# stone-d-chen/ffvvc

Measured on AMD Instinct MI355X. Metric: decoded frames/sec (4K/8K 10-bit VVC) per GPU, higher is better.
Workload: dtype u16

## Files before the change

ffvvc_amd/csrc/common.hpp:

```cpp
#pragma once
#include <hip/hip_runtime.h>
#include <stdint.h>
#include <stddef.h>
#include <stdio.h>
#include <stdlib.h>

#define VVC355_PB 128

namespace vvc355 { void hip_fail(const char *expr, int err, const char *what, const char *file, int line); }
#define HIP_CHECK(expr)                                                                         \
    do {                                                                                        \
        hipError_t e_ = (expr);                                                                 \
        if (e_ != hipSuccess)                                                                   \
            ::vvc355::hip_fail(#expr, (int)e_, hipGetErrorString(e_), __FILE__, __LINE__);      \
    } while (0)

namespace vvc355 {

template <int BD> struct Px       { using type = uint16_t; };
template <>       struct Px<8>    { using type = uint8_t;  };

__device__ __forceinline__ int clip3(int v, int lo, int hi) { return min(max(v, lo), hi); }
template <int BD> __device__ __forceinline__ int clip_px(int v) { return clip3(v, 0, (1 << BD) - 1); }
__device__ __forceinline__ int clip_intp2(int v, int p) { return clip3(v, -(1 << p), (1 << p) - 1); }
__device__ __forceinline__ int sign_of(int v) { return (v > 0) - (v < 0); }
__device__ __forceinline__ int ilog2(unsigned v) { return 31 - __clz(v | 1); }

#define VVC355_GLOBAL __attribute__((address_space(1)))
template <int N> struct RawBits;
template <> struct RawBits<1> { typedef uint8_t type; };
template <> struct RawBits<2> { typedef uint16_t type; };
template <> struct RawBits<4> { typedef uint32_t type; };
template <> struct RawBits<8> { typedef uint32_t type __attribute__((ext_vector_type(2))); };
template <> struct RawBits<16> { typedef uint32_t type __attribute__((ext_vector_type(4))); };
template <typename T> __device__ __forceinline__ T gld(const void *p)
{
    typedef typename RawBits<sizeof(T)>::type raw_t;
    const raw_t r = *(const VVC355_GLOBAL raw_t *)p;
    T v;
    __builtin_memcpy(&v, &r, sizeof(T));
    return v;
}
template <typename T> __device__ __forceinline__ void gst(void *p, T v)
{
    typedef typename RawBits<sizeof(T)>::type raw_t;
    raw_t r;
    __builtin_memcpy(&r, &v, sizeof(T));
    *(VVC355_GLOBAL raw_t *)p = r;
}

#define VVC355_CONST __attribute__((address_space(4)))
template <typename T> __device__ __forceinline__ T load_uniform(const T *p)
{
    static_assert(sizeof(T) % 4 == 0, "job descriptors are whole dwords");
    constexpr int N = sizeof(T) / 4;
    uint32_t w[N];
    const VVC355_CONST uint32_t *q = (const VVC355_CONST uint32_t *)p;
#pragma unroll
    for (int i = 0; i < N; i++) w[i] = q[i];
    T r;
    __builtin_memcpy(&r, w, sizeof(T));
    return r;
}

__device__ __forceinline__ ptrdiff_t row_off(int y, int stride) { return (ptrdiff_t)__mul24(y, stride); }

template <int BD> __device__ __forceinline__ int ld_px(const uint8_t *p, ptrdiff_t i)
{
    return ((const VVC355_GLOBAL typename Px<BD>::type *)p)[i];
}
template <int BD> __device__ __forceinline__ void st_px(uint8_t *p, ptrdiff_t i, int v)
{
    ((VVC355_GLOBAL typename Px<BD>::type *)p)[i] = (typename Px<BD>::type)v;
}

template <int BD> __device__ __forceinline__ int lmcs_fwd(const uint8_t *lut, int v)
{
    return lut ? (int)gld<typename Px<BD>::type>((const typename Px<BD>::type *)lut + v) : v;
}

template <typename T> __device__ __forceinline__ T gld_at(const uint8_t *base, uint32_t off) { return gld<T>(base + (size_t)off); }
template <typename T> __device__ __forceinline__ void gst_at(uint8_t *base, uint32_t off, T v) { gst<T>(base + (size_t)off, v); }

__device__ __forceinline__ int xcd_chunked(int b, int n)
{
    const int xcd = b & 7, idx = b >> 3, q = n >> 3, r = n & 7;
    return xcd * q + min(xcd, r) + idx;
}

__device__ __forceinline__ int xcd_grouped(int b, int n, int G)
{
    const int span = 8 * G, sg = b / span, r = b - sg * span;
    if ((sg + 1) * span > n)
        return b;
    return sg * span + (r & 7) * G + (r >> 3);
}

#define VVC355_BD_DISPATCH(bd, CALL)                         \
    do {                                                     \
        switch (bd) {                                        \
        case 8:  { constexpr int BD = 8;  CALL; } break;     \
        case 10: { constexpr int BD = 10; CALL; } break;     \
        case 12: { constexpr int BD = 12; CALL; } break;     \
        default:                                             \
            fprintf(stderr, "vvc_mi355: unsupported bit depth %d\n", (int)(bd)); abort(); \
        }                                                    \
    } while (0)

}
```

ffvvc_amd/csrc/inter_frame.hip:

```cpp
#include "common.hpp"
#include "inter_weight.hpp"
#include "runtime.hpp"
#include "../../include/vvc_mi355.h"

namespace vvc355 {

__global__ __launch_bounds__(256) void inter_build_kernel(const vvc355_inter_frame *__restrict__ fp)
{
    const vvc355_inter_frame f = load_uniform(fp);
    const int u = blockIdx.x * blockDim.x + threadIdx.x;
    if (u >= f.n_pus)
        return;
    const vvc355_inter_pu pu = ((const vvc355_inter_pu *)f.pus)[u];
    const vvc355_inter_slice *sl = (const vvc355_inter_slice *)f.slices + pu.slice;
    const vvc355_ref_pic *refs = (const vvc355_ref_pic *)f.refs;
    const MvFieldDev *mvf_tab = (const MvFieldDev *)f.mvf;
    vvc355_bipred_job *jl = (vvc355_bipred_job *)f.jobs_luma, *jc = (vvc355_bipred_job *)f.jobs_chroma;
    vvc355_bipred_result *rec = (vvc355_bipred_result *)f.records;
    const int sbw = pu.cb_width / pu.num_sb_x, sbh = pu.cb_height / pu.num_sb_y;
    const int tw = min(sbw, 16), th = min(sbh, 16);
    uint32_t job = pu.first_job;
    for (int sby = 0; sby < pu.num_sb_y; sby++)
        for (int sbx = 0; sbx < pu.num_sb_x; sbx++) {
            const int sx = pu.x0 + sbx * sbw, sy = pu.y0 + sby * sbh;
            const MvFieldDev mv = mvf_tab[(sy >> 2) * f.mvf_stride + (sx >> 2)];
            const bool bi = mv.pred_flag == 3;
            for (int ty = 0; ty < sbh; ty += th)
                for (int tx = 0; tx < sbw; tx += tw, job++) {
                    for (int c = 0; c < (f.chroma_format_idc ? 3 : 1); c++) {
                        const int hs = c ? f.hs : 0, vs = c ? f.vs : 0;
                        vvc355_bipred_job j = {};
                        const int x = (sx + tx) >> hs, y = (sy + ty) >> vs;
                        j.dst = f.dst[c] + (uint64_t)y * f.dst_stride[c] + ((uint64_t)x << f.pixel_shift);
                        j.dst_stride = f.dst_stride[c];
                        for (int l = 0; l < 2; l++) {
                            if (!(mv.pred_flag & (1 << l)))
                                continue;
                            const vvc355_ref_pic rp = refs[l * 16 + mv.ref_idx[l]];
                            (l ? j.ref1 : j.ref0) = rp.plane[c];
                            (l ? j.ref1_stride : j.ref0_stride) = rp.stride[c];
                            j.mv[2 * l] = mv.mv[l][0];
                            j.mv[2 * l + 1] = mv.mv[l][1];
                        }
                        j.rec = (uint64_t)(rec + job);
                        j.x = (int16_t)x; j.y = (int16_t)y; j.w = (int16_t)(tw >> hs); j.h = (int16_t)(th >> vs);
                        j.pic_w = (int16_t)(f.width >> hs); j.pic_h = (int16_t)(f.height >> vs);
                        j.chroma = c > 0; j.hs = f.hs; j.vs = f.vs;
                        j.dmvr = bi && pu.dmvr_flag;
                        j.bdof = !c && bi && pu.bdof_flag;
                        j.hf_idx = j.vf_idx = c ? 0 : pu.hpel_if_idx;
                        j.pred_flag = mv.pred_flag;
                        j.lmcs_lut = (!c && sl->lmcs_used && !pu.ciip_flag) ? f.lmcs_fwd_lut : 0;
                        set_pred_weight(j, derive_pred_weight(sl, mv, c, pu.dmvr_flag, pu.ciip_flag));
                        if (c == 0) jl[job] = j; else jc[2 * job + c - 1] = j;
                    }
                }
        }
}

__global__ __launch_bounds__(256) void inter_dmvr_info_kernel(const vvc355_inter_frame *__restrict__ fp)
{
    const vvc355_inter_frame f = load_uniform(fp);
    const int i = blockIdx.x * blockDim.x + threadIdx.x;
    if (i >= f.n_jobs)
        return;
    const vvc355_bipred_job *j = (const vvc355_bipred_job *)f.jobs_luma + i;
    if (!j->dmvr)
        return;
    const vvc355_bipred_result *r = (const vvc355_bipred_result *)f.records + i;
    const MvFieldDev *src = (const MvFieldDev *)f.mvf;
    MvFieldDev *dst = (MvFieldDev *)f.dmvr_mvf;
    MvFieldDev m = src[(j->y >> 2) * f.mvf_stride + (j->x >> 2)];
    m.mv[0][0] = r->mv[0]; m.mv[0][1] = r->mv[1]; m.mv[1][0] = r->mv[2]; m.mv[1][1] = r->mv[3];
    for (int y = j->y; y < j->y + j->h; y += 4)
        for (int x = j->x; x < j->x + j->w; x += 4)
            dst[(y >> 2) * f.mvf_stride + (x >> 2)] = m;
}

}

extern "C" {

void vvc355_inter_frame_build(void *stream, const vvc355_inter_frame *frame_dev, const vvc355_inter_frame *frame_host)
{
    if (frame_host->n_pus <= 0) return;
    hipLaunchKernelGGL(vvc355::inter_build_kernel, dim3((frame_host->n_pus + 255) / 256), dim3(256), 0, (hipStream_t)stream, frame_dev);
    HIP_CHECK(hipGetLastError());
}

void vvc355_inter_frame_pass(void *stream, int bd, const vvc355_inter_frame *frame_dev, const vvc355_inter_frame *frame_host)
{
    if (frame_host->n_pus <= 0 || frame_host->n_jobs <= 0) return;
    vvc355_inter_frame_build(stream, frame_dev, frame_host);
    vvc355_inter_frame_predict(stream, bd, frame_dev, frame_host);
}

void vvc355_inter_frame_predict(void *stream, int bd, const vvc355_inter_frame *frame_dev, const vvc355_inter_frame *frame_host)
{
    if (frame_host->n_pus <= 0 || frame_host->n_jobs <= 0) return;
    vvc355_bipred_batch(stream, bd, (const vvc355_bipred_job *)frame_host->jobs_luma, frame_host->n_jobs);
    if (frame_host->dmvr_mvf) {
        hipLaunchKernelGGL(vvc355::inter_dmvr_info_kernel, dim3((frame_host->n_jobs + 255) / 256), dim3(256), 0, (hipStream_t)stream, frame_dev);
        HIP_CHECK(hipGetLastError());
    }
    if (frame_host->chroma_format_idc)
        vvc355_bipred_chroma_batch(stream, bd, (const vvc355_bipred_job *)frame_host->jobs_chroma, 2 * frame_host->n_jobs);
}

}
```

ffvvc_amd/csrc/itx.hip:

```cpp
#include <type_traits>
#include "common.hpp"
#include "runtime.hpp"
#include "resid_math.hpp"
#include "../../include/vvc_mi355.h"
#include "stage_checks.hpp"

namespace vvc355 {

#define VVC355_TABLE(type, name, count) __device__ static const type d_tab_##name[count]
#include "tables.inc"
#undef VVC355_TABLE
#define VVC355_TABLE(type, name, count) static constexpr type c_##name[count]
#include "tables_small.inc"
#undef VVC355_TABLE
__host__ __device__ constexpr int level_scale_of(int rect, int rem)
{
    return rect ? (rem == 0 ? 57 : rem == 1 ? 64 : rem == 2 ? 72 : rem == 3 ? 80 : rem == 4 ? 90 : 102)
                : (rem == 0 ? 40 : rem == 1 ? 45 : rem == 2 ? 51 : rem == 3 ? 57 : rem == 4 ? 64 : 72);
}
static constexpr unsigned long long kDiag4X = 0x3323213210210100ull, kDiag4Y = 0x3231230123012010ull;
constexpr bool itx_small_tables_match()
{
    for (int r = 0; r < 2; r++)
        for (int q = 0; q < 6; q++)
// ... 408 lines not shown
            } else {
#pragma unroll
                for (int q = 0; q < PER; q++) {
                    const int o = e0 + q;
                    if (o < n)
                        st_px<BD>(dst + (ptrdiff_t)(o >> job.log2_w) * job.dst_stride, o & (w - 1), clip_px<BD>((int)pred[q] + r[q]));
                }
            }
        }
    }
}

template <int BD, int NT, int CAP, typename... Lv>
__global__ __launch_bounds__(256) void itx_kernel(const vvc355_itx_job *__restrict__ jobs, int n_jobs, Lv... lv)
{
    constexpr bool PACKED = sizeof...(Lv) > 0;
    constexpr int TBS = 256 / NT;
    __shared__ __attribute__((aligned(16))) int buf_all[TBS][CAP];
    __shared__ __attribute__((aligned(16))) int tmp_all[TBS][CAP];
    __shared__ int8_t cos_lds[256];
    cos_lds[threadIdx.x] = d_tab_dct2_cos[threadIdx.x];
    __syncthreads();
    const int sub = threadIdx.x / NT, tid = threadIdx.x % NT;
    const int ji = blockIdx.x * TBS + sub;
    if (ji >= n_jobs)
        return;
    vvc355_itx_job job = jobs[ji];
    resolve_type(job);
    if (job.log2_w + job.log2_h > __builtin_ctz(CAP))
        return;
    if constexpr (PACKED) {
        const LvSrc ls = lv_src(lv...);
        const vvc355_tb_levels r = ls.lv[ji];
        itx_generic_block<BD, NT, CAP, true>(job, buf_all[sub], tmp_all[sub], cos_lds, tid, &r, ls.levels);
    } else {
        itx_generic_block<BD, NT, CAP>(job, buf_all[sub], tmp_all[sub], cos_lds, tid);
    }
}


typedef short itx_v2s __attribute__((ext_vector_type(2)));
__device__ __forceinline__ int dot2_i16(uint32_t a, uint32_t b, int acc)
{
    return __builtin_amdgcn_sdot2(__builtin_bit_cast(itx_v2s, a), __builtin_bit_cast(itx_v2s, b), acc, false);
}
__device__ __forceinline__ uint32_t pack_i16(int lo, int hi) { return ((uint32_t)lo & 0xffffu) | ((uint32_t)hi << 16); }

template <int N> struct TxDim {
    static constexpr int KV = N < 32 ? N : 32;
    static constexpr int P = KV + (KV >= 16 ? 8 : 0);
    static constexpr int KS = KV < 8 ? 4 : 8;
    static constexpr int NTYPE = N <= 32 ? 3 : 1;
    __device__ static __forceinline__ const int16_t *table()
    {
        return N == 4 ? d_tab_itx16_4 : N == 8 ? d_tab_itx16_8 : N == 16 ? d_tab_itx16_16 : N == 32 ? d_tab_itx16_32 : d_tab_itx16_64;
    }
    __device__ static __forceinline__ void stage(int16_t *lds)
    {
        const int16_t *src = table();
        constexpr int ND = NTYPE * N * KV / 2;
        for (int i = threadIdx.x; i < ND; i += 256) {
            const int row = i / (KV / 2), c2 = i % (KV / 2);
            *(uint32_t *)&lds[row * P + 2 * c2] = gld<uint32_t>(src + 2 * i);
        }
    }
};

template <int KS> __device__ __forceinline__ void lds_row(const int16_t *p, uint32_t (&d)[KS / 2])
{
    if constexpr (KS == 8) {
        const uint4 v = *(const uint4 *)p;
        d[0] = v.x; d[1] = v.y; d[2] = v.z; d[3] = v.w;
    } else {
        const uint2 v = *(const uint2 *)p;
        d[0] = v.x; d[1] = v.y;
    }
}

template <int BD> __device__ __forceinline__ uint2 px4_load(const uint8_t *p)
{
    uint2 v = make_uint2(0, 0);
    if (BD > 8) v = gld<uint2>(p);
    else v.x = gld<uint32_t>(p);
    return v;
}
template <int BD> __device__ __forceinline__ void px4_add_store(uint8_t *p, uint2 praw, const int (&res)[4])
{
    if (BD > 8) {
        const int o0 = clip_px<BD>((int)(praw.x & 0xffff) + res[0]), o1 = clip_px<BD>((int)(praw.x >> 16) + res[1]);
        const int o2 = clip_px<BD>((int)(praw.y & 0xffff) + res[2]), o3 = clip_px<BD>((int)(praw.y >> 16) + res[3]);
        gst<uint2>(p, make_uint2((uint32_t)o0 | ((uint32_t)o1 << 16), (uint32_t)o2 | ((uint32_t)o3 << 16)));
    } else {
        const uint32_t pr = praw.x;
        const int o0 = clip_px<BD>((int)(pr & 0xff) + res[0]), o1 = clip_px<BD>((int)((pr >> 8) & 0xff) + res[1]);
        const int o2 = clip_px<BD>((int)((pr >> 16) & 0xff) + res[2]), o3 = clip_px<BD>((int)(pr >> 24) + res[3]);
        gst<uint32_t>(p, (uint32_t)o0 | ((uint32_t)o1 << 8) | ((uint32_t)o2 << 16) | ((uint32_t)o3 << 24));
    }
}

template <int BD, int LW, int LH, typename... Lv>
__global__ __launch_bounds__(256) void itx_shape_kernel(const vvc355_itx_job *__restrict__ jobs, int n_jobs, Lv... lv)
{
    constexpr bool PACKED = sizeof...(Lv) > 0;
#include "itx_shape_body.inc"
}

__global__ __launch_bounds__(256) void levels_expand_kernel(const vvc355_itx_job *__restrict__ jobs, LvSrc ls, int n_jobs)
{
    const int ji = blockIdx.x * 4 + (threadIdx.x >> 6), lane = threadIdx.x & 63;
    if (ji >= n_jobs)
        return;
    const vvc355_tb_levels r = ls.lv[ji];
    if (r.flags & VVC355_LEVELS_INT32)
        return;
    const vvc355_itx_job job = jobs[ji];
    int *coeffs = (int *)job.coeffs;
    const int lw = job.log2_w, w = 1 << lw;
    const int nzw = min((int)job.nzw, w), nzh = min((int)job.nzh, 1 << job.log2_h);
    const int sw = (nzw + 3) >> 2;
    for (int u = lane; u < sw * nzh; u += 64) {
        const int y = u / sw, x0 = (u - y * sw) * 4;
        const int16_t *g = lv_group(r, ls.levels, lw, x0, y);
        const int4 v = g ? unpack_i16x4(gld<uint2>(g + (y & 3) * 4)) : make_int4(0, 0, 0, 0);
        int *row = coeffs + y * w + x0;
        gst<int>(row, v.x);
        if (x0 + 1 < nzw) gst<int>(row + 1, v.y);
        if (x0 + 2 < nzw) gst<int>(row + 2, v.z);
        if (x0 + 3 < nzw) gst<int>(row + 3, v.w);
    }
}

__global__ __launch_bounds__(256) void dequant_kernel(const vvc355_dequant_job *__restrict__ jobs, int n_jobs)
{
    const int ji = blockIdx.x * 16 + (threadIdx.x >> 4), tid = threadIdx.x & 15;
    if (ji >= n_jobs)
        return;
    const vvc355_dequant_job job = jobs[ji];
    const int lw = job.log2_w;
    Dequant dq;
    dq.setup(1, lw, job.log2_h, job.qp, job.ts, job.dep_quant, job.bit_depth, job.range, (const uint8_t *)job.scale_matrix,
             job.log2_matrix_size, job.dc);
    const int rw = job.max_x - job.min_x + 1, rh = job.max_y - job.min_y + 1;
    int *coeffs = (int *)job.coeffs;
    const int cw = rw >= 16 ? 16 : rw > 8 ? 16 : rw > 4 ? 8 : rw > 2 ? 4 : rw > 1 ? 2 : 1;
    const int rows_per_pass = 16 / cw;
    for (int xb = 0; xb < rw; xb += 16) {
        const int xo = xb + (tid & (cw - 1));
        if (xo >= rw)
            continue;
        for (int yo = tid / cw; yo < rh; yo += rows_per_pass) {
            const int y = job.min_y + yo, x = job.min_x + xo;
            const int c = gld<int>(coeffs + (y << lw) + x);
            if (c)
                gst<int>(coeffs + (y << lw) + x, dq.apply(c, x, y));
        }
    }
}

template <int BD>
__global__ __launch_bounds__(256) void residual_kernel(const vvc355_blend_job *__restrict__ jobs)
{
    const vvc355_blend_job job = load_uniform(jobs + (blockIdx.y));
    int *res = (int *)job.src0;
    for (int i = blockIdx.x * blockDim.x + threadIdx.x; i < job.w * job.h; i += gridDim.x * blockDim.x) {
        int r = res[i];
        if (job.mode)
            r = (r * job.w0) >> job.denom;
        if (job.mode == 2) {
            res[i] = r;
            continue;
        }
        const int y = i / job.w, x = i - y * job.w;
        uint8_t *row = (uint8_t *)job.dst + (ptrdiff_t)y * job.dst_stride;
        st_px<BD>(row, x, clip_px<BD>(ld_px<BD>(row, x) + r));
    }
}

__global__ __launch_bounds__(128) void bdpcm_kernel(const vvc355_blend_job *__restrict__ jobs)
{
    const vvc355_blend_job job = load_uniform(jobs + (blockIdx.x));
    int *c = (int *)job.dst;
    const int w = job.w, h = job.h, range = job.denom, t = threadIdx.x;
    if (job.mode) {
        if (t < w)
            for (int y = 1; y < h; y++)
                c[y * w + t] = clip_intp2(c[y * w + t] + c[(y - 1) * w + t], range);
    } else {
        if (t < h)
            for (int x = 1; x < w; x++)
                c[t * w + x] = clip_intp2(c[t * w + x] + c[t * w + x - 1], range);
    }
}

__global__ __launch_bounds__(64) void lfnst_kernel(int *v, const int *u, int nz, int n_tr_s, int set, int idx, int range)
{
    const int j = threadIdx.x;
    if (j >= n_tr_s)
        return;
    const int8_t *m = n_tr_s > 16 ? d_tab_lfnst_8x8 + (set * 2 + idx - 1) * 16 * 48 : d_tab_lfnst_4x4 + (set * 2 + idx - 1) * 16 * 16;
    unsigned t = 0;
    for (int i = 0; i < nz; i++)
        t += (unsigned)u[i] * (unsigned)(int)m[i * n_tr_s + j];
    v[j] = clip_intp2(((int)t + 64) >> 7, range);
}

__global__ __launch_bounds__(256) void lfnst_batch_kernel(const vvc355_lfnst_job *__restrict__ jobs, int n_jobs)
{
    __shared__ int u_all[4][16];
    const int wave = threadIdx.x >> 6, lane = threadIdx.x & 63;
    const int ji = blockIdx.x * 4 + wave;
    if (ji >= n_jobs)
        return;
    const vvc355_lfnst_job job = jobs[ji];
    int *coeffs = (int *)job.coeffs;
    const int lw = job.log2_w, w = 1 << lw, h = 1 << job.log2_h;
    if (job.dequant) {
        Dequant dq;
        dq.setup(1, lw, job.log2_h, job.qp, 0, job.dep_quant, job.bit_depth, job.range, (const uint8_t *)job.scale_matrix, job.log2_matrix_size, job.dc);
        const int rw = job.max_x + 1, n = rw * (job.max_y + 1);
        for (int i = lane; i < n; i += 64) {
            const int y = i / rw, x = i - y * rw;
            const int c = gld<int>(coeffs + (y << lw) + x);
            if (c)
                gst<int>(coeffs + (y << lw) + x, dq.apply(c, x, y));
        }
        asm volatile("s_waitcnt vmcnt(0)" ::: "memory");
        __builtin_amdgcn_fence(__ATOMIC_ACQ_REL, "wavefront");
        __builtin_amdgcn_wave_barrier();
    }
    const bool big = w >= 8 && h >= 8;
    const int n_out = big ? 48 : 16;
    const int nz = ((w == 8 && h == 8) || (w == 4 && h == 4)) ? 8 : 16;
    const unsigned long long sx = kDiag4X, sy = kDiag4Y;
    if (lane < 16)
        u_all[wave][lane] = lane < nz ? gld<int>(coeffs + w * (int)((sy >> (4 * lane)) & 15) + (int)((sx >> (4 * lane)) & 15)) : 0;
    __builtin_amdgcn_fence(__ATOMIC_ACQ_REL, "wavefront");
    __builtin_amdgcn_wave_barrier();
    if (lane < n_out) {
        const int mode = job.pred_mode_intra;
        const int set = mode < 0 ? 1 : d_tab_lfnst_tr_set_index[mode];
        const int8_t *m = big ? d_tab_lfnst_8x8 + (set * 2 + job.lfnst_idx - 1) * 16 * 48 : d_tab_lfnst_4x4 + (set * 2 + job.lfnst_idx - 1) * 16 * 16;
        unsigned t = 0;
        for (int i = 0; i < nz; i++)
            t += (unsigned)u_all[wave][i] * (unsigned)(int)m[i * n_out + lane];
        const int v = clip_intp2(((int)t + 64) >> 7, job.range);
        int x, y;
        const int j = lane;
        if (mode > 34) {
            if (!big)        { y = j & 3; x = j >> 2; }
            else if (j < 32) { y = j & 7; x = j >> 3; }
            else             { y = (j - 32) & 3; x = 4 + ((j - 32) >> 2); }
        } else {
            if (!big)        { y = j >> 2; x = j & 3; }
            else if (j < 32) { y = j >> 3; x = j & 7; }
            else             { y = 4 + ((j - 32) >> 2); x = (j - 32) & 3; }
        }
        gst<int>(coeffs + y * w + x, v);
    }
}

static bool itx_entry_exists(int trh, int trv, int lw, int lh)
{
    if (lw < 0 || lh < 0 || lw > 6 || lh > 6 || trh < 0 || trh > 2 || trv < 0 || trv > 2 || (lw == 0 && lh == 0))
        return false;
    if (lh == 0) return trv == TX_DCT2 && (lw == 4 || lw == 5 || (lw == 6 && trh == TX_DCT2));
    if (lw == 0) return trh == TX_DCT2 && (lh == 4 || lh == 5 || (lh == 6 && trv == TX_DCT2));
    if (trh != TX_DCT2 && (lw < 2 || lw > 5)) return false;
    if (trv != TX_DCT2 && (lh < 2 || lh > 5)) return false;
    return true;
}

template <int BD, int LW, bool PACKED = false>
static void launch_itx_shape(hipStream_t st, const vvc355_itx_job *jobs_dev, int n_jobs, int log2_h, LvSrc ls = {})
{
#define VVC355_ITX_SHAPE(LH)                                                                                          \
    case LH: {                                                                                                        \
        constexpr int TBS = 256 / ((1 << (LW + LH)) / 16);                                                            \
        if constexpr (PACKED)                                                                                         \
            hipLaunchKernelGGL((itx_shape_kernel<BD, LW, LH, LvSrc>), dim3((n_jobs + TBS - 1) / TBS), dim3(256), 0, st, jobs_dev, n_jobs, ls); \
        else                                                                                                          \
            hipLaunchKernelGGL((itx_shape_kernel<BD, LW, LH>), dim3((n_jobs + TBS - 1) / TBS), dim3(256), 0, st, jobs_dev, n_jobs); \
    } break;
    switch (log2_h) {
    VVC355_ITX_SHAPE(2) VVC355_ITX_SHAPE(3) VVC355_ITX_SHAPE(4) VVC355_ITX_SHAPE(5) VVC355_ITX_SHAPE(6)
    }
#undef VVC355_ITX_SHAPE
}


template <int BD, bool PACKED = false>
static void launch_itx_shape_any(hipStream_t st, const vvc355_itx_job *jobs_dev, int n_jobs, int log2_w, int log2_h, LvSrc ls = {})
{
    switch (log2_w) {
    case 2: launch_itx_shape<BD, 2, PACKED>(st, jobs_dev, n_jobs, log2_h, ls); break;
    case 3: launch_itx_shape<BD, 3, PACKED>(st, jobs_dev, n_jobs, log2_h, ls); break;
    case 4: launch_itx_shape<BD, 4, PACKED>(st, jobs_dev, n_jobs, log2_h, ls); break;
    case 5: launch_itx_shape<BD, 5, PACKED>(st, jobs_dev, n_jobs, log2_h, ls); break;
    case 6: launch_itx_shape<BD, 6, PACKED>(st, jobs_dev, n_jobs, log2_h, ls); break;
    }
}

__global__ __launch_bounds__(256) void itx_build_kernel(const vvc355_itx_frame *__restrict__ fp)
{
    const vvc355_itx_frame f = load_uniform(fp);
    const int i = blockIdx.x * blockDim.x + threadIdx.x;
    if (i >= f.n_tus)
        return;
    const vvc355_itx_tu t = ((const vvc355_itx_tu *)f.tus)[i];
    vvc355_itx_job j = {};
    j.coeffs = f.coeffs + (uint64_t)t.coeff_off * 4;
    const int c = t.c_idx;
    const uint64_t plane = c == 0 ? f.plane[0] : c == 1 ? f.plane[1] : f.plane[2];
    const int stride = c == 0 ? f.stride[0] : c == 1 ? f.stride[1] : f.stride[2];
    const bool keep = (t.flags & 4) != 0;
    j.dst = keep ? 0 : plane + (uint64_t)t.y0 * stride + ((uint64_t)t.x0 << f.pixel_shift);
    j.dst_stride = stride;
    j.trh = t.tr & 15; j.trv = t.tr >> 4;
    j.log2_w = t.log2_w; j.log2_h = t.log2_h; j.nzw = t.nzw; j.nzh = t.nzh;
    j.range = f.range; j.bd = f.bd;
    j.store_coeffs = keep;
    j.dq_flags = (uint8_t)((t.flags & 1) | (t.flags & 2)); j.dq_qp = t.qp;
    j.log2_matrix_size = 1; j.dc = -1;
    j.mts_flags = (t.flags & 8) ? VVC355_ITX_DERIVE_TYPE : 0; j.tu_flags = f.tu_flags; j.c_idx = t.c_idx;
    ((vvc355_itx_job *)f.jobs)[i] = j;
    if (f.resid_jobs) {
        vvc355_lmcs_resid_job r = {};
        if (t.flags & 64) {
            r.dst = plane + (uint64_t)t.y0 * stride + ((uint64_t)t.x0 << f.pixel_shift);
            r.resid = j.coeffs; r.luma = f.plane[0];
            r.dst_stride = stride; r.luma_stride = f.stride[0];
            r.w = (int16_t)(1 << t.log2_w); r.h = (int16_t)(1 << t.log2_h);
            r.x_vpdu = (int16_t)((t.x0 << (c ? f.hs : 0)) & ~(f.size_y - 1)); r.y_vpdu = (int16_t)((t.y0 << (c ? f.vs : 0)) & ~(f.size_y - 1));
            r.pic_w = (int16_t)f.width; r.pic_h = (int16_t)f.height; r.size_y = f.size_y;
            r.avail_l = (t.flags >> 4) & 1; r.avail_t = (t.flags >> 5) & 1;
            r.joint = 8;
            if (f.scale_table) {
                const int ux = (f.width + f.size_y - 1) / f.size_y;
                r.luma = f.scale_table + (uint64_t)((r.y_vpdu / f.size_y) * ux + r.x_vpdu / f.size_y) * 2;
                r.joint = 8 | 16;
            }
        }
        ((vvc355_lmcs_resid_job *)f.resid_jobs)[i] = r;
    }
}

template <int NT, int CAP, bool PACKED>
__device__ __forceinline__ void intra_tb_group(const vvc355_intra_tb_frame &f, int first, int end, int wg, int *buf, int *tmp,
                                               const int8_t *cos_lds)
{
    constexpr int TBS = 256 / NT;
    const int sub = threadIdx.x / NT, tid = threadIdx.x % NT;
    const int i = first + wg * TBS + sub;
    if (i >= end)
        return;
    const vvc355_intra_tu t = ((const vvc355_intra_tu *)f.tus)[i];
    const int lw = t.log2_w, lh = t.log2_h;
    const bool lfnst = t.flags & VVC355_INTRA_TU_LFNST;
    if (lw + lh > __builtin_ctz(CAP) || lw + lh < 2 || lw > 6 || lh > 6 || (t.flags & ~(VVC355_INTRA_TU_DEP_QUANT | VVC355_INTRA_TU_LFNST)))
        return;
    if (lfnst && (lw < 2 || lh < 2 || t.lfnst_idx < 1 || t.lfnst_idx > 2 || t.pred_mode_intra > 94))
        return;
    vvc355_itx_job job = {};
    job.coeffs = f.coeffs + (uint64_t)t.coeff_off * 4;
    job.log2_w = t.log2_w; job.log2_h = t.log2_h;
    job.nzw = (uint8_t)min((int)t.nzw, 1 << lw); job.nzh = (uint8_t)min((int)t.nzh, 1 << lh);
    job.range = f.range; job.bd = f.bd;
    job.store_coeffs = 1;
    job.dq_flags = (uint8_t)(1 | ((t.flags & VVC355_INTRA_TU_DEP_QUANT) << 1)); job.dq_qp = t.qp;
    job.log2_matrix_size = 1; job.dc = -1;
    job.mts_flags = VVC355_ITX_DERIVE_TYPE; job.tu_flags = t.tu_flags; job.mts_idx = t.mts_idx; job.lfnst_idx = t.lfnst_idx; job.c_idx = t.c_idx;
    resolve_type(job);
    if constexpr (PACKED) {
        const vvc355_tb_levels r = ((const vvc355_tb_levels *)f.lv)[i];
        itx_generic_block<10, NT, CAP, true, true>(job, buf + sub * CAP, tmp + sub * CAP, cos_lds, tid, &r, (const int16_t *)f.levels,
                                                   lfnst ? t.lfnst_idx : 0, t.pred_mode_intra);
    } else {
        itx_generic_block<10, NT, CAP, false, true>(job, buf + sub * CAP, tmp + sub * CAP, cos_lds, tid, nullptr, nullptr,
                                                    lfnst ? t.lfnst_idx : 0, t.pred_mode_intra);
    }
}

template <int NT, int CAP, bool PACKED>
__global__ __launch_bounds__(256) void intra_tb_kernel(const vvc355_intra_tb_frame *__restrict__ fp, int first, int end)
{
    constexpr int TBS = 256 / NT;
    __shared__ __attribute__((aligned(16))) int buf_all[TBS * CAP];
    __shared__ __attribute__((aligned(16))) int tmp_all[TBS * CAP];
    __shared__ int8_t cos_lds[256];
    cos_lds[threadIdx.x] = d_tab_dct2_cos[threadIdx.x];
    __syncthreads();
    const vvc355_intra_tb_frame f = load_uniform(fp);
    intra_tb_group<NT, CAP, PACKED>(f, first, end, blockIdx.x, buf_all, tmp_all, cos_lds);
}

struct IntraTbGrid {
    int wg_first[4];
};
template <bool PACKED>
__global__ __launch_bounds__(256) void intra_tb_merged_kernel(const vvc355_intra_tb_frame *__restrict__ fp, IntraTbGrid g)
{
    __shared__ __attribute__((aligned(16))) int buf_all[1024];
    __shared__ __attribute__((aligned(16))) int tmp_all[1024];
    __shared__ int8_t cos_lds[256];
    cos_lds[threadIdx.x] = d_tab_dct2_cos[threadIdx.x];
    __syncthreads();
    const vvc355_intra_tb_frame f = load_uniform(fp);
    const int b = blockIdx.x;
    if (b < g.wg_first[0])
        intra_tb_group<4, 16, PACKED>(f, f.class_first[0], f.class_first[1], b, buf_all, tmp_all, cos_lds);
    else if (b < g.wg_first[1])
        intra_tb_group<16, 64, PACKED>(f, f.class_first[1], f.class_first[2], b - g.wg_first[0], buf_all, tmp_all, cos_lds);
    else if (b < g.wg_first[2])
        intra_tb_group<64, 256, PACKED>(f, f.class_first[2], f.class_first[3], b - g.wg_first[1], buf_all, tmp_all, cos_lds);
    else if (b < g.wg_first[3])
        intra_tb_group<256, 1024, PACKED>(f, f.class_first[3], f.class_first[4], b - g.wg_first[2], buf_all, tmp_all, cos_lds);
}

static constexpr int kIntraTbDefaultMode = 2;

template <bool PACKED>
static void launch_intra_tb(hipStream_t st, const vvc355_intra_tb_frame *fd, const vvc355_intra_tb_frame &fh, int mode)
{
    const int32_t *cf = fh.class_first;
    int wgs[5];
    for (int k = 0; k < 5; k++) {
        const int cnt = cf[k + 1] - cf[k], tbs = k == 0 ? 64 : k == 1 ? 16 : k == 2 ? 4 : 1;
        wgs[k] = (cnt + tbs - 1) / tbs;
    }
    if (mode == 2) {
        IntraTbGrid g;
        int total = 0;
        for (int k = 0; k < 4; k++)
            g.wg_first[k] = total += wgs[k];
        if (total)
            hipLaunchKernelGGL((intra_tb_merged_kernel<PACKED>), dim3(total), dim3(256), 0, st, fd, g);
    } else {
        if (wgs[0]) hipLaunchKernelGGL((intra_tb_kernel<4, 16, PACKED>), dim3(wgs[0]), dim3(256), 0, st, fd, cf[0], cf[1]);
        if (wgs[1]) hipLaunchKernelGGL((intra_tb_kernel<16, 64, PACKED>), dim3(wgs[1]), dim3(256), 0, st, fd, cf[1], cf[2]);
        if (wgs[2]) hipLaunchKernelGGL((intra_tb_kernel<64, 256, PACKED>), dim3(wgs[2]), dim3(256), 0, st, fd, cf[2], cf[3]);
        if (wgs[3]) hipLaunchKernelGGL((intra_tb_kernel<256, 1024, PACKED>), dim3(wgs[3]), dim3(256), 0, st, fd, cf[3], cf[4]);
    }
    if (wgs[4]) hipLaunchKernelGGL((intra_tb_kernel<256, 4096, PACKED>), dim3(wgs[4]), dim3(256), 0, st, fd, cf[4], cf[5]);
}

template <int BD> struct InterEpi {
    uint8_t *dst0, *dst1;
    int stride0, stride1;
    int *keep;
    int joint, scale;
    uint2 p0[4], p1[4];
    static constexpr int PXS = (int)sizeof(typename Px<BD>::type);
    __device__ __forceinline__ void prefetch(bool act, int x0, int y0)
    {
#pragma unroll
        for (int r = 0; r < 4; r++) {
            p0[r] = p1[r] = make_uint2(0, 0);
            if (act && !keep) {
                p0[r] = px4_load<BD>(dst0 + row_off(y0 + r, stride0) + x0 * PXS);
                if (dst1)
                    p1[r] = px4_load<BD>(dst1 + row_off(y0 + r, stride1) + x0 * PXS);
            }
        }
    }
    template <int W> __device__ __forceinline__ void row(int r, int x0, int y, const int (&res)[4])
    {
        if (keep) {
            gst<int4>(keep + y * W + x0, make_int4(res[0], res[1], res[2], res[3]));
            return;
        }
        int own[4], other[4];
#pragma unroll
        for (int q = 0; q < 4; q++) {
            own[q] = resid_sample<BD>(res[q], joint & 8, scale);
            other[q] = resid_sample<BD>(res[q], joint, scale);
        }
        px4_add_store<BD>(dst0 + row_off(y, stride0) + x0 * PXS, p0[r], own);
        if (dst1)
            px4_add_store<BD>(dst1 + row_off(y, stride1) + x0 * PXS, p1[r], other);
    }
    __device__ __forceinline__ void sample(int x, int y, int o, int r)
    {
        if (keep) {
            gst<int>(keep + o, r);
            return;
        }
        uint8_t *row0 = dst0 + row_off(y, stride0);
        st_px<BD>(row0, x, clip_px<BD>(ld_px<BD>(row0, x) + resid_sample<BD>(r, joint & 8, scale)));
        if (dst1) {
            uint8_t *row1 = dst1 + row_off(y, stride1);
            st_px<BD>(row1, x, clip_px<BD>(ld_px<BD>(row1, x) + resid_sample<BD>(r, joint, scale)));
        }
    }
};

struct InterTbHead {
    uint64_t tus, coeffs, lv, levels, plane[3], scale_table;
    int32_t  stride[3], width, height, n_tus;
    uint8_t  hs, vs, size_y, range, bd, pad_[3];
};
static_assert(sizeof(InterTbHead) == offsetof(vvc355_inter_tb_frame, bin_first) && offsetof(InterTbHead, hs) == offsetof(vvc355_inter_tb_frame, hs) &&
              offsetof(InterTbHead, stride) == offsetof(vvc355_inter_tb_frame, stride), "InterTbHead is the frame without bin_first");

template <int BD> struct InterTbSrc {
    using Epi = InterEpi<BD>;
    InterTbHead f;
    int first, ch, bin, lw0, lh0;
    __device__ __forceinline__ vvc355_tb_levels levels_of(int i) const
    {
        if (!f.lv)
            return vvc355_tb_levels{ 0, 0, VVC355_LEVELS_INT32 };
        const uint4 v = gld<uint4>((const vvc355_tb_levels *)f.lv + first + i);
        return vvc355_tb_levels{ (uint64_t)v.x | ((uint64_t)v.y << 32), v.z, v.w };
    }
    __device__ __forceinline__ const int16_t *stream() const { return (const int16_t *)f.levels; }
    __device__ __forceinline__ bool get(int i, vvc355_itx_job &job, Epi &epi) const
    {
        vvc355_inter_tu t;
        const uint4 raw = gld<uint4>((const vvc355_inter_tu *)f.tus + first + i);
        __builtin_memcpy(&t, &raw, sizeof(t));
        const int lw = t.log2_w, lh = t.log2_h, c = t.flags & 3, joint = t.joint_mts & 15, mts = (t.joint_mts >> 4) & 7;
        const bool keep = t.flags & VVC355_INTER_TU_KEEP;
        bool ok = lw <= 6 && lh <= 6 && lw + lh >= 2 && ((lw >= 2 && lh >= 2) ? (lw - 2) * 5 + (lh - 2) : 25) == bin;
        ok &= !(t.flags & 0xc0) && !(t.joint_mts & 0x80) && mts <= 4 && c != 3 && (c != 0) == (ch != 0) && !(c == 0 && joint);
        ok &= !((joint & 8) && !f.scale_table);
        const int hs = c ? f.hs : 0, vs = c ? f.vs : 0;
        ok &= t.x0 >= 0 && t.y0 >= 0 && t.x0 + (1 << (lw & 7)) <= (f.width >> hs) && t.y0 + (1 << (lh & 7)) <= (f.height >> vs);
        if (keep || (levels_of(i).flags & VVC355_LEVELS_INT32))
            ok &= !(t.coeff_off & 3);
        int scale = 0;
        if (ok && (joint & 8)) {
            const int ls = f.size_y == 64 ? 6 : 5;
            const int ux = ((t.x0 << hs) >> ls) - ((t.flags >> 4) & 1), uy = ((t.y0 << vs) >> ls) - ((t.flags >> 5) & 1);
            ok = ux >= 0 && uy >= 0;
            if (ok)
                scale = (int)gld<int16_t>((const int16_t *)f.scale_table + uy * ((f.width + (1 << ls) - 1) >> ls) + ux);
        }
        job = {};
        job.log2_w = (uint8_t)(ok ? lw : lw0); job.log2_h = (uint8_t)(ok ? lh : lh0);
        job.nzw = job.nzh = 1;
        job.range = f.range; job.bd = f.bd;
        job.log2_matrix_size = 1; job.dc = -1;
        epi.dst0 = epi.dst1 = nullptr;
        epi.keep = nullptr;
        epi.stride0 = epi.stride1 = 0;
        epi.joint = epi.scale = 0;
        if (!ok)
            return false;
        job.coeffs = f.coeffs + (uint64_t)t.coeff_off * 4;
        job.nzw = (uint8_t)min((int)t.nzw, 1 << lw); job.nzh = (uint8_t)min((int)t.nzh, 1 << lh);
        job.dq_flags = (uint8_t)(1 | ((t.flags & VVC355_INTER_TU_DEP_QUANT) ? 2 : 0)); job.dq_qp = t.qp;
        job.mts_flags = VVC355_ITX_DERIVE_TYPE; job.tu_flags = t.tu_flags; job.mts_idx = (uint8_t)mts; job.c_idx = (uint8_t)c;
        resolve_type(job);
        if (((lw < 2 || lw > 5) && job.trh) || ((lh < 2 || lh > 5) && job.trv)) {
            job.trh = job.trv = 0;
            return false;
        }
        const uint64_t p0 = f.plane[0], p1 = f.plane[1], p2 = f.plane[2];
        const int s0 = f.stride[0], s1 = f.stride[1], s2 = f.stride[2];
        const uint64_t plane = c == 0 ? p0 : c == 1 ? p1 : p2, other = c == 1 ? p2 : p1;
        const int stride = c == 0 ? s0 : c == 1 ? s1 : s2, ostride = c == 1 ? s2 : s1;
        if (keep) {
            epi.keep = (int *)job.coeffs;
            return true;
        }
        epi.dst0 = (uint8_t *)plane + row_off(t.y0, stride) + t.x0 * Epi::PXS;
        epi.stride0 = stride;
        if (joint & 1) {
            epi.dst1 = (uint8_t *)other + row_off(t.y0, ostride) + t.x0 * Epi::PXS;
            epi.stride1 = ostride;
        }
        epi.joint = joint;
        epi.scale = scale;
        return true;
    }
};

template <int BD, int LW, int LH>
__global__ __launch_bounds__(256) void inter_tb_shape_kernel(const vvc355_inter_tb_frame *__restrict__ fp, int first, int end, int ch)
{
    constexpr bool PACKED = true;
    const InterTbSrc<BD> src{ load_uniform((const InterTbHead *)fp), first, ch, (LW - 2) * 5 + (LH - 2), LW, LH };
    const int n_jobs = end - first;
#define ITX_SHAPE_RECORDS
#include "itx_shape_body.inc"
#undef ITX_SHAPE_RECORDS
}
#undef ITX_SYNC

template <int BD>
__global__ __launch_bounds__(256) void inter_tb_thin_kernel(const vvc355_inter_tb_frame *__restrict__ fp, int first, int end, int ch)
{
    __shared__ __attribute__((aligned(16))) int buf_all[4 * 256];
    __shared__ __attribute__((aligned(16))) int tmp_all[4 * 256];
    __shared__ int8_t cos_lds[256];
    cos_lds[threadIdx.x] = d_tab_dct2_cos[threadIdx.x];
    __syncthreads();
    const int sub = threadIdx.x >> 6, tid = threadIdx.x & 63;
    const int i = xcd_chunked(blockIdx.x, gridDim.x) * 4 + sub;
    if (i >= end - first)
        return;
    const InterTbSrc<BD> src{ load_uniform((const InterTbHead *)fp), first, ch, 25, 1, 1 };
    vvc355_itx_job job;
    InterEpi<BD> epi;
    if (!src.get(i, job, epi))
        return;
    const vvc355_tb_levels r = src.levels_of(i);
    itx_generic_block<BD, 64, 256, true, false, InterEpi<BD>>(job, buf_all + sub * 256, tmp_all + sub * 256, cos_lds, tid, &r, src.stream(), 0, 0, &epi);
}

template <int BD, int LW>
static void launch_inter_tb_shape(hipStream_t st, const vvc355_inter_tb_frame *fd, int first, int end, int ch, int log2_h)
{
#define VVC355_INTER_TB_SHAPE(LH)                                                                                     \
    case LH: {                                                                                                        \
        constexpr int TBS = 256 / ((1 << (LW + LH)) / 16);                                                            \
        hipLaunchKernelGGL((inter_tb_shape_kernel<BD, LW, LH>), dim3((end - first + TBS - 1) / TBS), dim3(256), 0, st, fd, first, end, ch); \
    } break;
    switch (log2_h) {
    VVC355_INTER_TB_SHAPE(2) VVC355_INTER_TB_SHAPE(3) VVC355_INTER_TB_SHAPE(4) VVC355_INTER_TB_SHAPE(5) VVC355_INTER_TB_SHAPE(6)
    }
#undef VVC355_INTER_TB_SHAPE
}

template <int BD>
static void launch_inter_tb(hipStream_t st, const vvc355_inter_tb_frame *fd, const vvc355_inter_tb_frame &fh, int channels)
{
    for (int ch = 0; ch < 2; ch++) {
        if (!(channels & (1 << ch)))
            continue;
        for (int bin = 0; bin < VVC355_INTER_TB_BINS; bin++) {
            const int first = fh.bin_first[ch][bin], end = fh.bin_first[ch][bin + 1];
            if (end <= first)
                continue;
            if (bin == 25) {
                hipLaunchKernelGGL((inter_tb_thin_kernel<BD>), dim3((end - first + 3) / 4), dim3(256), 0, st, fd, first, end, ch);
                continue;
            }
            switch (bin / 5 + 2) {
            case 2: launch_inter_tb_shape<BD, 2>(st, fd, first, end, ch, bin % 5 + 2); break;
            case 3: launch_inter_tb_shape<BD, 3>(st, fd, first, end, ch, bin % 5 + 2); break;
            case 4: launch_inter_tb_shape<BD, 4>(st, fd, first, end, ch, bin % 5 + 2); break;
            case 5: launch_inter_tb_shape<BD, 5>(st, fd, first, end, ch, bin % 5 + 2); break;
            case 6: launch_inter_tb_shape<BD, 6>(st, fd, first, end, ch, bin % 5 + 2); break;
            }
        }
    }
// ... 563 lines not shown
```

Before: 595.2.

## Stage job descriptors in LDS for coalesced stores and flatten inter build per tile

Job-build kernels for inter prediction and inverse transform now write each job struct into padded shared-memory rows and then copy them to global memory with coalesced 8-byte stores, rather than each thread writing a large strided struct on its own. The inter builder also caches the reference table and PU headers in LDS and maps one lane to each tile job through a binary search over job offsets, with separate waves for luma and the two chroma planes. The goal is better parallelism when PUs contain many sub-block jobs. The cost is extra LDS usage, barriers and search work, plus a fallback path when job ranges are not contiguous.

```diff
diff --git a/ffvvc_amd/csrc/common.hpp b/ffvvc_amd/csrc/common.hpp
--- a/ffvvc_amd/csrc/common.hpp
+++ b/ffvvc_amd/csrc/common.hpp
@@ -82,6 +82,23 @@
 template <typename T> __device__ __forceinline__ T gld_at(const uint8_t *base, uint32_t off) { return gld<T>(base + (size_t)off); }
 template <typename T> __device__ __forceinline__ void gst_at(uint8_t *base, uint32_t off, T v) { gst<T>(base + (size_t)off, v); }
 
+template <int PITCH, typename T> __device__ __forceinline__ void lds_row_put(uint32_t *rows, int r, const T &v)
+{
+    static_assert(sizeof(T) % 8 == 0 && PITCH % 2 == 1 && PITCH * 4 > (int)sizeof(T), "whole 8-byte pairs, odd pitch");
+    uint32_t w[sizeof(T) / 4];
+    __builtin_memcpy(w, &v, sizeof(T));
+#pragma unroll
+    for (int k = 0; k < (int)(sizeof(T) / 4); k++) rows[r * PITCH + k] = w[k];
+}
+template <int N, int PITCH> __device__ __forceinline__ void lds_rows_to_global(const uint32_t *rows, void *dst, int n_rows)
+{
+    static_assert(N % 2 == 0 && PITCH % 2 == 1 && PITCH > N, "whole 8-byte pairs, odd pitch");
+    for (int p = threadIdx.x; p < n_rows * (N / 2); p += blockDim.x) {
+        const int r = p / (N / 2), k = 2 * (p - r * (N / 2));
+        gst<uint2>((uint8_t *)dst + (size_t)p * 8, make_uint2(rows[r * PITCH + k], rows[r * PITCH + k + 1]));
+    }
+}
+
 __device__ __forceinline__ int xcd_chunked(int b, int n)
 {
     const int xcd = b & 7, idx = b >> 3, q = n >> 3, r = n & 7;
diff --git a/ffvvc_amd/csrc/inter_frame.hip b/ffvvc_amd/csrc/inter_frame.hip
--- a/ffvvc_amd/csrc/inter_frame.hip
+++ b/ffvvc_amd/csrc/inter_frame.hip
@@ -5,57 +5,153 @@
 
 namespace vvc355 {
 
-__global__ __launch_bounds__(256) void inter_build_kernel(const vvc355_inter_frame *__restrict__ fp)
-{
-    const vvc355_inter_frame f = load_uniform(fp);
-    const int u = blockIdx.x * blockDim.x + threadIdx.x;
-    if (u >= f.n_pus)
-        return;
-    const vvc355_inter_pu pu = ((const vvc355_inter_pu *)f.pus)[u];
+struct RefMem {
+    const vvc355_ref_pic *t;
+    __device__ __forceinline__ uint64_t plane(int i, int c) const { return t[i].plane[c]; }
+    __device__ __forceinline__ int stride(int i, int c) const { return t[i].stride[c]; }
+};
+struct RefLds {
+    static constexpr int DW = sizeof(vvc355_ref_pic) / 4;
+    const uint32_t *t;
+    __device__ __forceinline__ uint64_t plane(int i, int c) const { return t[i * DW + 2 * c] | (uint64_t)t[i * DW + 2 * c + 1] << 32; }
+    __device__ __forceinline__ int stride(int i, int c) const { return (int)t[i * DW + 6 + c]; }
+};
+
+template <typename Refs>
+__device__ __forceinline__ vvc355_bipred_job inter_tile_job(const vvc355_inter_frame &f, const vvc355_inter_pu &pu, const vvc355_inter_slice *sl,
+                                                            const MvFieldDev &mv, const Refs &refs, int c, uint32_t job, int px, int py, int tw, int th)
+{
+    const int hs = c ? f.hs : 0, vs = c ? f.vs : 0;
+    const bool bi = mv.pred_flag == 3;
+    vvc355_bipred_job j = {};
+    const int x = px >> hs, y = py >> vs;
+    j.dst = f.dst[c] + (uint64_t)y * f.dst_stride[c] + ((uint64_t)x << f.pixel_shift);
+    j.dst_stride = f.dst_stride[c];
+    for (int l = 0; l < 2; l++) {
+        if (!(mv.pred_flag & (1 << l)))
+            continue;
+        const int r = l * 16 + (mv.ref_idx[l] & 15);
+        (l ? j.ref1 : j.ref0) = refs.plane(r, c);
+        (l ? j.ref1_stride : j.ref0_stride) = refs.stride(r, c);
+        j.mv[2 * l] = mv.mv[l][0];
+        j.mv[2 * l + 1] = mv.mv[l][1];
+    }
+    j.rec = (uint64_t)((vvc355_bipred_result *)f.records + job);
+    j.x = (int16_t)x; j.y = (int16_t)y; j.w = (int16_t)(tw >> hs); j.h = (int16_t)(th >> vs);
+    j.pic_w = (int16_t)(f.width >> hs); j.pic_h = (int16_t)(f.height >> vs);
+    j.chroma = c > 0; j.hs = f.hs; j.vs = f.vs;
+    j.dmvr = bi && pu.dmvr_flag;
+    j.bdof = !c && bi && pu.bdof_flag;
+    j.hf_idx = j.vf_idx = c ? 0 : pu.hpel_if_idx;
+    j.pred_flag = mv.pred_flag;
+    j.lmcs_lut = (!c && sl->lmcs_used && !pu.ciip_flag) ? f.lmcs_fwd_lut : 0;
+    set_pred_weight(j, derive_pred_weight(sl, mv, c, pu.dmvr_flag, pu.ciip_flag));
+    return j;
+}
+
+__device__ __forceinline__ MvFieldDev load_mvf(const vvc355_inter_frame &f, int sx, int sy)
+{
+    const uint32_t *p = (const uint32_t *)((const MvFieldDev *)f.mvf + ((sy >> 2) * f.mvf_stride + (sx >> 2)));
+    uint32_t w[sizeof(MvFieldDev) / 4];
+#pragma unroll
+    for (int k = 0; k < (int)(sizeof(MvFieldDev) / 4); k++) w[k] = gld<uint32_t>(p + k);
+    MvFieldDev mv;
+    __builtin_memcpy(&mv, w, sizeof(mv));
+    return mv;
+}
+
+__device__ void inter_build_unit(const vvc355_inter_frame &f, const vvc355_inter_pu &pu)
+{
     const vvc355_inter_slice *sl = (const vvc355_inter_slice *)f.slices + pu.slice;
-    const vvc355_ref_pic *refs = (const vvc355_ref_pic *)f.refs;
-    const MvFieldDev *mvf_tab = (const MvFieldDev *)f.mvf;
+    const RefMem refs = { (const vvc355_ref_pic *)f.refs };
     vvc355_bipred_job *jl = (vvc355_bipred_job *)f.jobs_luma, *jc = (vvc355_bipred_job *)f.jobs_chroma;
-    vvc355_bipred_result *rec = (vvc355_bipred_result *)f.records;
     const int sbw = pu.cb_width / pu.num_sb_x, sbh = pu.cb_height / pu.num_sb_y;
     const int tw = min(sbw, 16), th = min(sbh, 16);
     uint32_t job = pu.first_job;
     for (int sby = 0; sby < pu.num_sb_y; sby++)
         for (int sbx = 0; sbx < pu.num_sb_x; sbx++) {
             const int sx = pu.x0 + sbx * sbw, sy = pu.y0 + sby * sbh;
-            const MvFieldDev mv = mvf_tab[(sy >> 2) * f.mvf_stride + (sx >> 2)];
-            const bool bi = mv.pred_flag == 3;
+            const MvFieldDev mv = load_mvf(f, sx, sy);
             for (int ty = 0; ty < sbh; ty += th)
                 for (int tx = 0; tx < sbw; tx += tw, job++) {
-                    for (int c = 0; c < (f.chroma_format_idc ? 3 : 1); c++) {
-                        const int hs = c ? f.hs : 0, vs = c ? f.vs : 0;
-                        vvc355_bipred_job j = {};
-                        const int x = (sx + tx) >> hs, y = (sy + ty) >> vs;
-                        j.dst = f.dst[c] + (uint64_t)y * f.dst_stride[c] + ((uint64_t)x << f.pixel_shift);
-                        j.dst_stride = f.dst_stride[c];
-                        for (int l = 0; l < 2; l++) {
-                            if (!(mv.pred_flag & (1 << l)))
-                                continue;
-                            const vvc355_ref_pic rp = refs[l * 16 + mv.ref_idx[l]];
-                            (l ? j.ref1 : j.ref0) = rp.plane[c];
-                            (l ? j.ref1_stride : j.ref0_stride) = rp.stride[c];
-                            j.mv[2 * l] = mv.mv[l][0];
-                            j.mv[2 * l + 1] = mv.mv[l][1];
-                        }
-                        j.rec = (uint64_t)(rec + job);
-                        j.x = (int16_t)x; j.y = (int16_t)y; j.w = (int16_t)(tw >> hs); j.h = (int16_t)(th >> vs);
-                        j.pic_w = (int16_t)(f.width >> hs); j.pic_h = (int16_t)(f.height >> vs);
-                        j.chroma = c > 0; j.hs = f.hs; j.vs = f.vs;
-                        j.dmvr = bi && pu.dmvr_flag;
-                        j.bdof = !c && bi && pu.bdof_flag;
-                        j.hf_idx = j.vf_idx = c ? 0 : pu.hpel_if_idx;
-                        j.pred_flag = mv.pred_flag;
-                        j.lmcs_lut = (!c && sl->lmcs_used && !pu.ciip_flag) ? f.lmcs_fwd_lut : 0;
-                        set_pred_weight(j, derive_pred_weight(sl, mv, c, pu.dmvr_flag, pu.ciip_flag));
-                        if (c == 0) jl[job] = j; else jc[2 * job + c - 1] = j;
-                    }
+                    jl[job] = inter_tile_job(f, pu, sl, mv, refs, 0, job, sx + tx, sy + ty, tw, th);
+                    if (!f.chroma_format_idc)
+                        continue;
+                    jc[2 * job] = inter_tile_job(f, pu, sl, mv, refs, 1, job, sx + tx, sy + ty, tw, th);
+                    jc[2 * job + 1] = inter_tile_job(f, pu, sl, mv, refs, 2, job, sx + tx, sy + ty, tw, th);
                 }
         }
+}
+
+constexpr int kInterBuildUnits = 64;
+__global__ __launch_bounds__(256) void inter_build_kernel(const vvc355_inter_frame *__restrict__ fp)
+{
+    constexpr int WG = 256, U = kInterBuildUnits, CH = 64, JOB_DW = sizeof(vvc355_bipred_job) / 4, PITCH = JOB_DW + 1, PU_DW = sizeof(vvc355_inter_pu) / 4;
+    constexpr int REF_DW = 32 * RefLds::DW;
+    static_assert(JOB_DW == 26 && PU_DW == 5 && RefLds::DW == 10, "row pitches below are odd");
+    __shared__ uint32_t s_luma[CH * PITCH], s_chroma[2 * CH * PITCH];
+    __shared__ uint32_t s_pu[(U + 1) * PU_DW];
+    __shared__ uint32_t s_refs[REF_DW];
+    const vvc355_inter_frame f = load_uniform(fp);
+    const int tid = threadIdx.x, wave = tid / 64, lane = tid % 64, u0 = blockIdx.x * U, nu = min(U, f.n_pus - u0);
+    for (int k = tid; k < REF_DW; k += WG)
+        s_refs[k] = gld<uint32_t>((const uint32_t *)f.refs + k);
+    vvc355_inter_pu own = {};
+    uint32_t own_end = 0;
+    if (tid < nu) {
+        uint32_t w[PU_DW];
+#pragma unroll
+        for (int k = 0; k < PU_DW; k++) s_pu[tid * PU_DW + k] = w[k] = gld<uint32_t>((const uint32_t *)f.pus + (size_t)(u0 + tid) * PU_DW + k);
+        __builtin_memcpy(&own, w, sizeof(own));
+        const int sbw = own.cb_width / own.num_sb_x, sbh = own.cb_height / own.num_sb_y;
+        own_end = own.first_job + own.num_sb_x * own.num_sb_y * ((sbw + 15) / 16) * ((sbh + 15) / 16);
+        if (tid == nu - 1)
+            s_pu[nu * PU_DW + 4] = own_end;
+    }
+    __syncthreads();
+    if (!__syncthreads_and(tid >= nu || s_pu[(tid + 1) * PU_DW + 4] == own_end)) {
+        if (tid < nu)
+            inter_build_unit(f, own);
+        return;
+    }
+    const RefLds refs = { s_refs };
+    const uint32_t first = s_pu[4], total = s_pu[nu * PU_DW + 4] - first;
+    const int ncomp = f.chroma_format_idc ? 3 : 1;
+    for (uint32_t c0 = 0; c0 < total; c0 += CH) {
+        const int n = (int)min((uint32_t)CH, total - c0);
+        if (wave < ncomp && lane < n) {
+            const uint32_t job = first + c0 + lane;
+            int lo = 0, hi = nu;
+            while (hi - lo > 1) {
+                const int mid = (lo + hi) >> 1;
+                if (s_pu[mid * PU_DW + 4] <= job) lo = mid; else hi = mid;
+            }
+            uint32_t w[PU_DW];
+#pragma unroll
+            for (int k = 0; k < PU_DW; k++) w[k] = s_pu[lo * PU_DW + k];
+            vvc355_inter_pu pu;
+            __builtin_memcpy(&pu, w, sizeof(pu));
+            const vvc355_inter_slice *sl = (const vvc355_inter_slice *)f.slices + pu.slice;
+            const int sbw = pu.cb_width / pu.num_sb_x, sbh = pu.cb_height / pu.num_sb_y;
+            const int tw = min(sbw, 16), th = min(sbh, 16);
+            const int ntx = (sbw + 15) / 16, nty = (sbh + 15) / 16;
+            const int local = (int)(job - pu.first_job), sb = local / (ntx * nty), t = local - sb * (ntx * nty);
+            const int sby = sb / pu.num_sb_x, sbx = sb - sby * pu.num_sb_x, ty = t / ntx, tx = t - ty * ntx;
+            const int sx = pu.x0 + sbx * sbw, sy = pu.y0 + sby * sbh, px = sx + tx * tw, py = sy + ty * th;
+            const MvFieldDev mv = load_mvf(f, sx, sy);
+            if (wave == 0)
+                lds_row_put<PITCH>(s_luma, lane, inter_tile_job(f, pu, sl, mv, refs, 0, job, px, py, tw, th));
+            else if (wave == 1)
+                lds_row_put<PITCH>(s_chroma, 2 * lane, inter_tile_job(f, pu, sl, mv, refs, 1, job, px, py, tw, th));
+            else
+                lds_row_put<PITCH>(s_chroma, 2 * lane + 1, inter_tile_job(f, pu, sl, mv, refs, 2, job, px, py, tw, th));
+        }
+        __syncthreads();
+        lds_rows_to_global<JOB_DW, PITCH>(s_luma, (vvc355_bipred_job *)f.jobs_luma + (first + c0), n);
+        if (f.chroma_format_idc)
+            lds_rows_to_global<JOB_DW, PITCH>(s_chroma, (vvc355_bipred_job *)f.jobs_chroma + 2 * (size_t)(first + c0), 2 * n);
+        __syncthreads();
+    }
 }
 
 __global__ __launch_bounds__(256) void inter_dmvr_info_kernel(const vvc355_inter_frame *__restrict__ fp)
@@ -84,7 +180,8 @@
 void vvc355_inter_frame_build(void *stream, const vvc355_inter_frame *frame_dev, const vvc355_inter_frame *frame_host)
 {
     if (frame_host->n_pus <= 0) return;
-    hipLaunchKernelGGL(vvc355::inter_build_kernel, dim3((frame_host->n_pus + 255) / 256), dim3(256), 0, (hipStream_t)stream, frame_dev);
+    hipLaunchKernelGGL(vvc355::inter_build_kernel, dim3((frame_host->n_pus + vvc355::kInterBuildUnits - 1) / vvc355::kInterBuildUnits), dim3(256), 0,
+                       (hipStream_t)stream, frame_dev);
     HIP_CHECK(hipGetLastError());
 }
 
diff --git a/ffvvc_amd/csrc/itx.hip b/ffvvc_amd/csrc/itx.hip
--- a/ffvvc_amd/csrc/itx.hip
+++ b/ffvvc_amd/csrc/itx.hip
@@ -734,46 +734,56 @@
 
 __global__ __launch_bounds__(256) void itx_build_kernel(const vvc355_itx_frame *__restrict__ fp)
 {
+    constexpr int WG = 256, JOB_DW = sizeof(vvc355_itx_job) / 4, RES_DW = sizeof(vvc355_lmcs_resid_job) / 4;
+    __shared__ uint32_t s_jobs[WG * (JOB_DW + 1)], s_resid[WG * (RES_DW + 1)];
     const vvc355_itx_frame f = load_uniform(fp);
-    const int i = blockIdx.x * blockDim.x + threadIdx.x;
-    if (i >= f.n_tus)
-        return;
-    const vvc355_itx_tu t = ((const vvc355_itx_tu *)f.tus)[i];
-    vvc355_itx_job j = {};
-    j.coeffs = f.coeffs + (uint64_t)t.coeff_off * 4;
-    const int c = t.c_idx;
-    const uint64_t plane = c == 0 ? f.plane[0] : c == 1 ? f.plane[1] : f.plane[2];
-    const int stride = c == 0 ? f.stride[0] : c == 1 ? f.stride[1] : f.stride[2];
-    const bool keep = (t.flags & 4) != 0;
-    j.dst = keep ? 0 : plane + (uint64_t)t.y0 * stride + ((uint64_t)t.x0 << f.pixel_shift);
-    j.dst_stride = stride;
-    j.trh = t.tr & 15; j.trv = t.tr >> 4;
-    j.log2_w = t.log2_w; j.log2_h = t.log2_h; j.nzw = t.nzw; j.nzh = t.nzh;
-    j.range = f.range; j.bd = f.bd;
-    j.store_coeffs = keep;
-    j.dq_flags = (uint8_t)((t.flags & 1) | (t.flags & 2)); j.dq_qp = t.qp;
-    j.log2_matrix_size = 1; j.dc = -1;
-    j.mts_flags = (t.flags & 8) ? VVC355_ITX_DERIVE_TYPE : 0; j.tu_flags = f.tu_flags; j.c_idx = t.c_idx;
-    ((vvc355_itx_job *)f.jobs)[i] = j;
-    if (f.resid_jobs) {
-        vvc355_lmcs_resid_job r = {};
-        if (t.flags & 64) {
-            r.dst = plane + (uint64_t)t.y0 * stride + ((uint64_t)t.x0 << f.pixel_shift);
-            r.resid = j.coeffs; r.luma = f.plane[0];
-            r.dst_stride = stride; r.luma_stride = f.stride[0];
-            r.w = (int16_t)(1 << t.log2_w); r.h = (int16_t)(1 << t.log2_h);
-            r.x_vpdu = (int16_t)((t.x0 << (c ? f.hs : 0)) & ~(f.size_y - 1)); r.y_vpdu = (int16_t)((t.y0 << (c ? f.vs : 0)) & ~(f.size_y - 1));
-            r.pic_w = (int16_t)f.width; r.pic_h = (int16_t)f.height; r.size_y = f.size_y;
-            r.avail_l = (t.flags >> 4) & 1; r.avail_t = (t.flags >> 5) & 1;
-            r.joint = 8;
-            if (f.scale_table) {
-                const int ux = (f.width + f.size_y - 1) / f.size_y;
-                r.luma = f.scale_table + (uint64_t)((r.y_vpdu / f.size_y) * ux + r.x_vpdu / f.size_y) * 2;
-                r.joint = 8 | 16;
-            }
-        }
-        ((vvc355_lmcs_resid_job *)f.resid_jobs)[i] = r;
-    }
+    const int tid = threadIdx.x, first = blockIdx.x * WG, n = min(WG, f.n_tus - first);
+    if (tid < n) {
+        uint32_t tw[sizeof(vvc355_itx_tu) / 4];
+#pragma unroll
+        for (int k = 0; k < 4; k++) tw[k] = gld<uint32_t>((const uint32_t *)f.tus + (size_t)(first + tid) * 4 + k);
+        vvc355_itx_tu t;
+        __builtin_memcpy(&t, tw, sizeof(t));
+        vvc355_itx_job j = {};
+        j.coeffs = f.coeffs + (uint64_t)t.coeff_off * 4;
+        const int c = t.c_idx;
+        const uint64_t plane = c == 0 ? f.plane[0] : c == 1 ? f.plane[1] : f.plane[2];
+        const int stride = c == 0 ? f.stride[0] : c == 1 ? f.stride[1] : f.stride[2];
+        const bool keep = (t.flags & 4) != 0;
+        j.dst = keep ? 0 : plane + (uint64_t)t.y0 * stride + ((uint64_t)t.x0 << f.pixel_shift);
+        j.dst_stride = stride;
+        j.trh = t.tr & 15; j.trv = t.tr >> 4;
+        j.log2_w = t.log2_w; j.log2_h = t.log2_h; j.nzw = t.nzw; j.nzh = t.nzh;
+        j.range = f.range; j.bd = f.bd;
+        j.store_coeffs = keep;
+        j.dq_flags = (uint8_t)((t.flags & 1) | (t.flags & 2)); j.dq_qp = t.qp;
+        j.log2_matrix_size = 1; j.dc = -1;
+        j.mts_flags = (t.flags & 8) ? VVC355_ITX_DERIVE_TYPE : 0; j.tu_flags = f.tu_flags; j.c_idx = t.c_idx;
+        lds_row_put<JOB_DW + 1>(s_jobs, tid, j);
+        if (f.resid_jobs) {
+            vvc355_lmcs_resid_job r = {};
+            if (t.flags & 64) {
+                r.dst = plane + (uint64_t)t.y0 * stride + ((uint64_t)t.x0 << f.pixel_shift);
+                r.resid = j.coeffs; r.luma = f.plane[0];
+                r.dst_stride = stride; r.luma_stride = f.stride[0];
+                r.w = (int16_t)(1 << t.log2_w); r.h = (int16_t)(1 << t.log2_h);
+                r.x_vpdu = (int16_t)((t.x0 << (c ? f.hs : 0)) & ~(f.size_y - 1)); r.y_vpdu = (int16_t)((t.y0 << (c ? f.vs : 0)) & ~(f.size_y - 1));
+                r.pic_w = (int16_t)f.width; r.pic_h = (int16_t)f.height; r.size_y = f.size_y;
+                r.avail_l = (t.flags >> 4) & 1; r.avail_t = (t.flags >> 5) & 1;
+                r.joint = 8;
+                if (f.scale_table) {
+                    const int ux = (f.width + f.size_y - 1) / f.size_y;
+                    r.luma = f.scale_table + (uint64_t)((r.y_vpdu / f.size_y) * ux + r.x_vpdu / f.size_y) * 2;
+                    r.joint = 8 | 16;
+                }
+            }
+            lds_row_put<RES_DW + 1>(s_resid, tid, r);
+        }
+    }
+    __syncthreads();
+    lds_rows_to_global<JOB_DW, JOB_DW + 1>(s_jobs, (vvc355_itx_job *)f.jobs + first, n);
+    if (f.resid_jobs)
+        lds_rows_to_global<RES_DW, RES_DW + 1>(s_resid, (vvc355_lmcs_resid_job *)f.resid_jobs + first, n);
 }
 
 template <int NT, int CAP, bool PACKED>
```

After: 603.5 (median of 6 runs). +1.4%, better.
